# bobwan1995/cliora

Measured on AMD Instinct MI355X. Metric: sentences/sec (inside+outside fwd+bwd), len-20 d=400 bsz=64, higher is better.
Workload: dtype f32 (compose GEMMs: 3x bf16 MFMA per product, fp32 accumulate)

## Files before the change

cliora_amd/csrc/api_common.hpp:

```cpp
#pragma once
#include <hip/hip_runtime.h>
#include <hip/hip_ext.h>

#include <algorithm>
#include <cstdio>
#include <cstdlib>
#include <cstring>
#include <mutex>
#include <new>
#include <string>
#include <vector>

#include "../../include/cliora_chart.h"
#include "chart_kernels.hpp"
#include "gemm_kernels.hpp"
#include "wgrad_tiles.hpp"
#include "plan.hpp"

using namespace cliora;

struct cliora_plan {
    Plan p;
    bool uploaded = false;
    int device = -1;
// ... 170 lines not shown
enum { IMG_NONE = 0, IMG_FRAG_F32 = 2 };

template <class AP, class EP>
static int launch_rows_direct(hipStream_t st, const float* W, const float* img, int kind, int K, int ncols, int nrows, AP ap, EP ep) {
    if (nrows <= 0) return CLIORA_OK;
    const int nt = ncols / 16;
    if (kind == IMG_FRAG_F32) return launch_ksplit_f32<true>(st, img, K, nt, nrows, ap, ep);
    return launch_ksplit_f32<false>(st, W, K, nt, nrows, ap, ep);
}

template <class AP, class EP>
static int launch_rows(hipStream_t st, const float* W, int Kseg, int nseg, int ncols, int nrows, AP ap, EP ep) {
    if (nrows <= 0) return CLIORA_OK;
    const size_t budget = 150 * 1024;
    const int nt = ncols / 16;
    for (int ct : {5, 4, 2, 1}) {
        if (nt % ct) continue;
        if ((size_t)ct * 16 * (Kseg + WS_LDS_PAD) * sizeof(float) > budget) continue;
        switch (ct) {
            case 5: return launch_rows_ct<5>(st, W, Kseg, nseg, ncols, nrows, ap, ep);
            case 4: return launch_rows_ct<4>(st, W, Kseg, nseg, ncols, nrows, ap, ep);
            case 2: return launch_rows_ct<2>(st, W, Kseg, nseg, ncols, nrows, ap, ep);
            default: return launch_rows_ct<1>(st, W, Kseg, nseg, ncols, nrows, ap, ep);
        }
    }
    return fail(CLIORA_EINVAL, "weight block does not fit LDS");
}

constexpr int TN_DIRECT_ROWS = 4096;
constexpr int TN_DIRECT_BLOCKS = 256;

template <int T, class AP, class BP>
static int launch_tn_t(hipStream_t st, int nrows, int Mi, int Nj, AP ap, BP bp, float* slab, size_t slab_floats,
                       float* out, float* colsum_out, int accumulate) {
    const int blocks = (Mi / (T * 16)) * (Nj / (T * 16));
    size_t per_slice = (size_t)Mi * Nj + (colsum_out ? Mi : 0);
    int nsl = (int)std::min<size_t>(slab_floats / per_slice, (size_t)std::max(1, 2048 / blocks));
    nsl = std::min(nsl, (nrows + 15) / 16);
    nsl = std::max(4, nsl / 4 * 4);
    if ((size_t)nsl * per_slice > slab_floats) return fail(CLIORA_ENOMEM, "slab too small for the weight-gradient GEMM");
    int rps = (nrows + nsl - 1) / nsl;
    rps = (rps + 3) / 4 * 4;
    float* csl = slab + (size_t)nsl * Mi * Nj;
    if (colsum_out)
        hipLaunchKernelGGL((tn_gemm<T, T, true, AP, BP>), dim3(blocks, nsl / 4), dim3(WS_THREADS), 0, st, nrows, rps, Mi, Nj, ap, bp, slab, csl);
    else
        hipLaunchKernelGGL((tn_gemm<T, T, false, AP, BP>), dim3(blocks, nsl / 4), dim3(WS_THREADS), 0, st, nrows, rps, Mi, Nj, ap, bp, slab, csl);
    LAUNCHOK("tn_gemm");
    const size_t n = (size_t)Mi * Nj;
    launch_slab_reduce(st, slab, nsl, n, out, accumulate, csl, (size_t)Mi, colsum_out);
    LAUNCHOK("slab_reduce");
    return CLIORA_OK;
}

template <class AP, class BP>
static int launch_tn(hipStream_t st, int nrows, int Mi, int Nj, int Dp, AP ap, BP bp, float* slab, size_t slab_floats,
                     float* out, float* colsum_out, int accumulate = 0) {
    if (nrows <= 0) {
        if (accumulate) return CLIORA_OK;
        HIPOK(hipMemsetAsync(out, 0, (size_t)Mi * Nj * sizeof(float), st));
        if (colsum_out) HIPOK(hipMemsetAsync(colsum_out, 0, (size_t)Mi * sizeof(float), st));
        return CLIORA_OK;
    }
    if (nrows <= TN_DIRECT_ROWS && (Mi / 16) * (Nj / 16) <= TN_DIRECT_BLOCKS) {
        const int blocks = (Mi / 16) * (Nj / 16);
        if (colsum_out)
            hipLaunchKernelGGL((tn_gemm_direct<true, AP, BP>), dim3(blocks), dim3(TND_WAVES * 64), 0, st, nrows, Mi, Nj, ap, bp, out, colsum_out, accumulate);
        else
            hipLaunchKernelGGL((tn_gemm_direct<false, AP, BP>), dim3(blocks), dim3(TND_WAVES * 64), 0, st, nrows, Mi, Nj, ap, bp, out, colsum_out, accumulate);
        LAUNCHOK("tn_gemm_direct");
        return CLIORA_OK;
    }
    switch (pick_tiles(Dp / 16)) {
        case 5: return launch_tn_t<5>(st, nrows, Mi, Nj, ap, bp, slab, slab_floats, out, colsum_out, accumulate);
        case 4: return launch_tn_t<4>(st, nrows, Mi, Nj, ap, bp, slab, slab_floats, out, colsum_out, accumulate);
        case 2: return launch_tn_t<2>(st, nrows, Mi, Nj, ap, bp, slab, slab_floats, out, colsum_out, accumulate);
        default: return launch_tn_t<1>(st, nrows, Mi, Nj, ap, bp, slab, slab_floats, out, colsum_out, accumulate);
    }
}

template <int NIT, int NJT>
static int launch_tn_pairs_inst(hipStream_t st, const float* DZ, const float* X, int nrows, int Dp, int nkb, float* slab,
                                size_t slab_floats, float* out, float* colsum_out, int accumulate, int slices_cap, int ldz, int ldx) {
    const size_t per_slice = (size_t)Dp * Dp + Dp;
    int nsl = (int)std::min<size_t>(slab_floats / per_slice, (size_t)std::max(1, 256 / nkb));
    nsl = std::max(1, std::min(nsl, (nrows + 63) / 64));
    int rps = (nrows + nsl - 1) / nsl;
    rps = (rps + TN_RS - 1) / TN_RS * TN_RS;
    nsl = (nrows + rps - 1) / rps;
    float* csl = slab + (size_t)nsl * Dp * Dp;
    const size_t lds3 = (size_t)2 * TN3_RS * (Dp + NJT * 16) * sizeof(float) + (size_t)NJT * 2048;
    const bool strided = ldz != Dp || ldx != Dp;
    if (split_bf16() && lds3 <= 160 * 1024 && (Dp + NJT * 16) / 32 <= TN3_NP) {
        const int nsl_cap = slices_cap > 0 ? slices_cap : std::max(1, 230 / (8 * nkb)) * 8;
        if (nsl > nsl_cap) { nsl = nsl_cap; rps = (nrows + nsl - 1) / nsl; }
        rps = (rps + TN3_RS - 1) / TN3_RS * TN3_RS;
        nsl = (nrows + rps - 1) / rps;
        csl = slab + (size_t)nsl * Dp * Dp;
        if constexpr (NIT == 7 && NJT == 9) {
            OKR(cliora_ensure_max_lds((const void*)tn_gemm_dma3x<NIT, NJT, 5, true>));
            hipLaunchKernelGGL((tn_gemm_dma3x<NIT, NJT, 5, true>), dim3(8 * nkb * ((nsl + 7) / 8)), dim3(512), lds3, st, DZ, ldz, X, ldx, nrows, rps, nsl, Dp, Dp, nkb, slab, csl);
            LAUNCHOK("tn_gemm_dma3x");
        } else {
            if (strided) return fail(CLIORA_EINVAL, "strided operands need the eight-wave weight-gradient kernel (tn_pairs_strided_ok)");
            OKR(cliora_ensure_max_lds((const void*)tn_gemm_dma3<NIT, NJT, true>));
            hipLaunchKernelGGL((tn_gemm_dma3<NIT, NJT, true>), dim3(8 * nkb * ((nsl + 7) / 8)), dim3(256), lds3, st, DZ, X, nrows, rps, nsl, Dp, Dp, nkb, slab, csl);
            LAUNCHOK("tn_gemm_dma3");
        }
    } else {
        if (strided) return fail(CLIORA_EINVAL, "strided operands need the eight-wave weight-gradient kernel (tn_pairs_strided_ok)");
// ... 5 lines not shown
    const size_t n = (size_t)Dp * Dp;
    launch_slab_reduce(st, slab, nsl, n, out, accumulate, csl, (size_t)Dp, colsum_out);
    LAUNCHOK("slab_reduce");
    return CLIORA_OK;
}

static bool tn_pairs_two_ranges_ok(int Dp) {
    const int NT = Dp / 16;
    return split_bf16() && NT > 20 && NT <= 27;
}
static int launch_tn_pairs_two_ranges(hipStream_t st, const float* DZ, const float* X, int n1, long long start2, int n2, int Dp, float* slab,
                                      size_t slab_floats, float* out, float* colsum_out, int slices_cap) {
    constexpr int NIT = 7, NJT = 9, nkb = 3;
    const size_t per_slice = (size_t)Dp * Dp + Dp;
    const size_t lds3 = (size_t)2 * TN3_RS * (Dp + NJT * 16) * sizeof(float) + (size_t)NJT * 2048;
    int cap = std::min<int>((int)(slab_floats / per_slice), slices_cap > 0 ? slices_cap : std::max(1, 230 / (8 * nkb)) * 8);
    cap = std::max(2, cap);
    int rps = (n1 + n2 + cap - 1) / cap;
    rps = (rps + TN3_RS - 1) / TN3_RS * TN3_RS;
    int s1 = (n1 + rps - 1) / rps, s2 = (n2 + rps - 1) / rps;
    while (s1 + s2 > cap) { rps += TN3_RS; s1 = (n1 + rps - 1) / rps; s2 = (n2 + rps - 1) / rps; }
    const int nsl = s1 + s2;
    float* csl = slab + (size_t)nsl * Dp * Dp;
    OKR(cliora_ensure_max_lds((const void*)tn_gemm_dma3x<NIT, NJT, 5, true>));
    hipLaunchKernelGGL((tn_gemm_dma3x<NIT, NJT, 5, true>), dim3(8 * nkb * ((nsl + 7) / 8)), dim3(512), lds3, st, DZ, Dp, X, Dp, n1, rps, nsl, Dp, Dp, nkb,
                       slab, csl, s1, n2, start2);
    LAUNCHOK("tn_gemm_dma3x(two ranges)");
    launch_slab_reduce(st, slab, nsl, (size_t)Dp * Dp, out, 0, csl, (size_t)Dp, colsum_out);
    LAUNCHOK("slab_reduce");
    return CLIORA_OK;
}

static int launch_tn_level_block(hipStream_t st, const float* A, int lda, const float* Bm, int nsent, int C, int off, int hi, int Dp,
                                 float* slab, size_t slab_floats, float* out, float* colsum_out, int accumulate, int slices_cap, int nblk) {
    constexpr int NIT = 7, NJT = 9, nkb = 3;
    const int nrows = nsent * hi;
    if (nrows <= 0) return CLIORA_OK;
    const size_t per_slice = ((size_t)Dp * Dp + Dp) * nblk;
    const size_t lds3 = (size_t)2 * TN3_RS * (Dp + NJT * 16) * sizeof(float) + (size_t)NJT * 2048;
    int cap = std::min<int>((int)(slab_floats / per_slice), slices_cap > 0 ? slices_cap : std::max(1, 230 / (8 * nkb)) * 8);
    cap = std::max(1, std::min(cap, (nrows + 63) / 64));
    int rps = (nrows + cap - 1) / cap;
    rps = (rps + TN3_RS - 1) / TN3_RS * TN3_RS;
    const int nsl = (nrows + rps - 1) / rps;
    float* csl = slab + (size_t)nsl * nblk * Dp * Dp;
    OKR(cliora_ensure_max_lds((const void*)tn_gemm_dma3x<NIT, NJT, 5, true>));
    hipLaunchKernelGGL((tn_gemm_dma3x<NIT, NJT, 5, true>), dim3(8 * nkb * ((nsl + 7) / 8), nblk), dim3(512), lds3, st, A, lda, Bm, Dp, nrows, rps, nsl,
                       Dp, Dp, nkb, slab, csl, 0x7fffffff, 0, 0LL, hi, C, off, (long long)Dp);
    LAUNCHOK("tn_gemm_dma3x(level rows)");
    launch_slab_reduce(st, slab, nsl, (size_t)nblk * Dp * Dp, out, accumulate, csl, (size_t)nblk * Dp, colsum_out);
    LAUNCHOK("slab_reduce");
    return CLIORA_OK;
}

static bool pair_tiles_ok(int Dp) {
    return split_bf16() && Dp == 400;
}
static int launch_tn_tiles(hipStream_t st, const float* DZt, const float* Xt, long long tile0, long long ntiles, long long tile0b, long long ntilesb,
                           int Dp, float* slab, size_t slab_floats, float* out, float* colsum_out, int accumulate, int slices_cap) {
    const int NT = Dp / 16;
    const long long nt = ntiles + ntilesb;
    if (nt <= 0) {
        if (accumulate) return CLIORA_OK;
        HIPOK(hipMemsetAsync(out, 0, (size_t)Dp * Dp * sizeof(float), st));
        if (colsum_out) HIPOK(hipMemsetAsync(colsum_out, 0, (size_t)Dp * sizeof(float), st));
        return CLIORA_OK;
    }
    constexpr int NTc = 25, NIT = 7, NJT = 9, NJW = 5, nkb = 3;
    if (NT != NTc) return fail(CLIORA_EINVAL, "tiled pair-row operands: d = 400 only");
    const size_t per_slice = (size_t)Dp * Dp + Dp;
    long long cap = std::min<long long>((long long)(slab_floats / per_slice), slices_cap > 0 ? slices_cap : std::max(1, 230 / (8 * nkb)) * 8);
    cap = std::max<long long>(2, std::min(cap, (nt + 3) / 4));
    long long tps = (nt + cap - 1) / cap;
    tps = (tps + 1) / 2 * 2;
    long long s1 = (ntiles + tps - 1) / tps, s2 = (ntilesb + tps - 1) / tps;
    while (s1 + s2 > cap) { tps += 2; s1 = (ntiles + tps - 1) / tps; s2 = (ntilesb + tps - 1) / tps; }
    const int nsl = (int)(s1 + s2);
    float* csl = slab + (size_t)nsl * Dp * Dp;
    const size_t lds = (size_t)2 * 2048 * (NT + NJT) + 1024;
    OKR(cliora_ensure_max_lds((const void*)tn_gemm_tiles<NTc, NIT, NJT, NJW, true>));
    hipLaunchKernelGGL((tn_gemm_tiles<NTc, NIT, NJT, NJW, true>), dim3(8 * nkb * ((nsl + 7) / 8)), dim3(512), lds, st, reinterpret_cast<const uint32_t*>(DZt),
                       reinterpret_cast<const uint32_t*>(Xt), tile0, (int)ntiles, (int)tps, nsl, nkb, slab, csl, (int)s1, tile0b, (int)ntilesb);
// ... 198 lines not shown
```

cliora_amd/csrc/api_mlp.hip:

```cpp
#include "api_common.hpp"
#include <hip/hip_ext.h>
#include "level_kernels.hpp"
#include "ragged_kernels.hpp"
#include "resident_kernels.hpp"
#include "vl_kernels.hpp"

#define ATTEND_LAUNCH(kern, R_, grid, stream, ...)                                                              \
    do {                                                                                                      \
        if ((R_) <= 36) hipLaunchKernelGGL(kern<9>, grid, dim3(256), 0, stream, __VA_ARGS__);                  \
        else hipLaunchKernelGGL(kern<16>, grid, dim3(256), 0, stream, __VA_ARGS__);                            \
    } while (0)

struct ComposeLaunch { int TG, SP, ntask, gx; };
static ComposeLaunch compose_launch(const cliora_plan* plan, int level, bool outside_pass) {
    const Plan& p = plan->p;
    const int32_t* e = p.level_geom.data() + ((size_t)(outside_pass ? p.L : 0) + level) * PLEVEL_INTS;
    ComposeLaunch q{e[5], e[6], e[7], std::min(e[7], p.compose_cap)};
    if (q.gx >= 8 && (q.gx + 7) / 8 * 8 <= p.compose_cap) q.gx = (q.gx + 7) / 8 * 8;
    return q;
}

static size_t compose_lds_bytes(int ct, int S, bool with_slots) {
    return (size_t)ct * 16 * S * sizeof(uint32_t) + (with_slots ? (size_t)LC_SLOTS * ct * 64 * sizeof(float4) : 0);
}
// ... 680 lines not shown
        if (level == L - 1) {
            if (compress) {
                hipLaunchKernelGGL(cell_dnorm, dim3(cells_grid(ncell)), dim3(256), 0, sb, g, VHo, OH, ws + f.nrmo, p.normalize, dGo);
                LAUNCHOK("cell_dnorm(root)");
                return CLIORA_OK;
            }
            LAUNCH_SIGNALLING(done, root_bwd, dim3(1), dim3(ROOT_WAVES * 64), 0, sb, B, C, Dp, VHo, OH, ws + f.nrmo, p.normalize, wb + bw.groot);
            LAUNCHOK("root_bwd");
            return CLIORA_OK;
        }
        if (!fused_norm) {
            hipLaunchKernelGGL(cell_dnorm, dim3(cells_grid(ncell)), dim3(256), 0, sb, g, VHo, OH, ws + f.nrmo, p.normalize, dGo);
            LAUNCHOK("cell_dnorm(out)");
        }
        {
            ProfScope ps(CLIORA_KCLASS_COMPOSE_BWD, sb);
            OKR(launch_level_compose_bwd(sb, ws + f.w2oT, ws + f.w2oT3, f.S3, Dp, f.ct3, f.ncb3, pair_level(level, true), dGo, YM, Pp,
                                         PI + (size_t)p.blk_plo * Dp, ldpi, ws + f.po, Dp, ws + f.b2o, DA, DZ, Xp, DPP, DPB, tiled));
        }
        const bool sib_last = sibling_runs(L - 2 - level);
        LAUNCH_SIGNALLING(sib_last ? nullptr : done, cell_dsoftmax, dim3(cells_grid(ncell)), dim3(256), 0, sb, g, f.ncb3, DPP, DPB, Sp, Pp, OS, dStoto, DS);
        LAUNCHOK("cell_dsoftmax(out)");
        OKR(sibling_gather(L - 2 - level, done));
        return CLIORA_OK;
    };

    static const int ksplit_env = [] { const char* e = getenv("CLIORA_WGRAD_SPLIT_LEVEL"); return e ? atoi(e) : -1; }();
    const bool wcat_split_path = split_bf16() && tn_pairs_strided_ok(Dp);
    const bool sw_beside = plan->side2_beside;
    const int ksplit = ksplit_env >= 0 ? ksplit_env : !sw_beside ? 0
                     : wcat_split_path ? std::max(1, std::min(2 * L / 5, L - 1)) : std::min(2, L - 1);
    int tail_cells = C;
    bool dpi_done_recorded = false;
    auto wcat_grad = [&](hipStream_t s_, int off, int hi, int accumulate) -> int {
        if (tn_pairs_strided_ok(Dp) && (long long)B * hi >= 512 && (long long)B * hi < (1LL << 22)) {
            return launch_tn_level_block(s_, dPI, ldpi, IH, B, C, off, hi, Dp, wb + bw.slab2, bw.slab_floats, wb + bw.gwcat, wb + bw.gbcat, accumulate,
                                         std::max(8, (180 / (3 * nb)) / 4 * 4), nb);
        }
        return launch_tn(s_, B * hi, ldpi, Dp, Dp, LevelRowsA{dPI, ldpi, C, off, hi}, LevelRowsA{IH, Dp, C, off, hi}, wb + bw.slab2,
                         bw.slab_floats, wb + bw.gwcat, wb + bw.gbcat, accumulate);
    };
    auto inside_bwd_step = [&](int level) -> int {
        const LevelArgs g = level_args(p, level, false);
        const int ncell = B * g.Lc;
        const bool fused_norm = fuse_dnorm && p.share && !vl && level >= 1 && level <= L - 2;
        hipLaunchKernelGGL(cell_gather_bwd_in, dim3(ncell), dim3(256), 0, sa, g, D, d_inside_h,
                           level == 0 ? nullptr : d_inside_s, dv.use[ROLE_INA], dv.use[ROLE_INB], dv.use[ROLE_OUTA],
                           !ran_outside ? 0 : (sib_on_outside_chain(level) ? 1 : 2),
                           sibPL, sibQL, ldsib, wb + bw.sib_s, DA, DS, PI, ldpi, p.share, IH, OH, dPI, VH, dStot,
                           ws + f.bcat, fused_norm ? wb + bw.dots : nullptr);
        LAUNCHOK("cell_gather_bwd_in");
        if (level == 0) {
            HIPOK(hipEventRecord(plan->ev_fork[2], sa));
            dpi_done_recorded = true;
        }
        if (fused_norm && gemm3)
            OKR(launch_rows_direct3x(sa, ws + f.wcatT3s, ldpi, Dp, ncell, LevelRowsA{dPI, ldpi, C, g.off, g.Lc},
                              NormBwdLevelE{dG, VH, IH, ws + f.nrmi, wb + bw.dots, Dp, C, g.off, g.Lc, p.normalize}, bwd_gemm3));
        else if (fused_norm)
            OKR(launch_rows_direct(sa, ws + f.wcatT, PROJ_IMG(f.wcatT3), ldpi, Dp, ncell, LevelRowsA{dPI, ldpi, C, g.off, g.Lc},
                            NormBwdLevelE{dG, VH, IH, ws + f.nrmi, wb + bw.dots, Dp, C, g.off, g.Lc, p.normalize}));
        else if (level <= L - 2 && gemm3)
            OKR(launch_rows_direct3x(sa, ws + f.wcatT3s, ldpi, Dp, ncell, LevelRowsA{dPI, ldpi, C, g.off, g.Lc},
                              StoreLevelE{VH, Dp, C, g.off, g.Lc, nullptr, 1}, bwd_gemm3));
        else if (level <= L - 2)
            OKR(launch_rows_direct(sa, ws + f.wcatT, PROJ_IMG(f.wcatT3), ldpi, Dp, ncell, LevelRowsA{dPI, ldpi, C, g.off, g.Lc},
                            StoreLevelE{VH, Dp, C, g.off, g.Lc, nullptr, 1}));
        else if (compress && ran_outside)
            OKR(launch_rows_direct(sa, ws + f.rootwT, PROJ_IMG(f.rootwT3), Dp, Dp, ncell, LevelRowsA{dGo, Dp, C, g.off, g.Lc},
                            StoreLevelE{VH, Dp, C, g.off, g.Lc, nullptr, 1}));
        if (vl) {
            ATTEND_LAUNCH(cell_attend_bwd, p.R, dim3(ncell), sa, g, VH, IH, ws + f.nrmi, p.normalize, OBJ, p.R,
                               drop_mask, ws + f.att_pk, wb + bw.dctx, wb + bw.pmo, wb + bw.dsc, IHn, nrmIn, level >= 1 ? dG : (float*)nullptr);
            LAUNCHOK("cell_attend_bwd");
        }
        if (level == ksplit && level >= 1) {
            const int hi = tail_cells - g.off;
            HIPOK(hipEventRecord(plan->ev_fork[2], sa));
            HIPOK(hipStreamWaitEvent(sw, plan->ev_fork[2], 0));
            OKR(wcat_grad(sw, g.off, hi, tail_cells < C));
            tail_cells = g.off;
        }
        if (level == 0) return CLIORA_OK;
        if (!fused_norm && !vl) {
            hipLaunchKernelGGL(cell_dnorm, dim3(cells_grid(ncell)), dim3(256), 0, sa, g, VH, IHn, nrmIn, p.normalize, dG);
            LAUNCHOK("cell_dnorm(in)");
        }
        {
// ... 60 lines not shown
        }
        if (two_streams && j >= 1) HIPOK(hipStreamWaitEvent(sa, plan->ev_level[j - 1], 0));
        OKR(inside_bwd_step(L - 1 - j));
        if (j == J_early) {
            early_r0 = p.row_base_in(L - 1 - j);
            early_r1 = p.row_base_out(j + 1);
            HIPOK(hipEventRecord(plan->ev_fork[2], sa));
            HIPOK(hipStreamWaitEvent(sw, plan->ev_fork[2], 0));
            if (two_streams) HIPOK(hipStreamWaitEvent(sw, plan->ev_level[j], 0));
            early_t0 = p.tile_base_in(L - 1 - j);
            early_t1 = p.tile_base_out(j + 1);
            if (tiled)
                OKR(launch_tn_tiles(sw, DZ, Xp, early_t0, early_t1 - early_t0, 0, 0, Dp, wb + bw.slab2, bw.slab_floats, wb + bw.gw2o, wb + bw.gb2o, 0,
                                    early_slices));
            else
                OKR(launch_tn_pairs(sw, DZ + (size_t)early_r0 * Dp, Xp + (size_t)early_r0 * Dp, (int)(early_r1 - early_r0), Dp, wb + bw.slab2, bw.slab_floats,
                                    wb + bw.gw2o, wb + bw.gb2o, 0, early_slices));
        }
        if (tiled && J_early >= 0 && j == J_early2) {
            const long long t0 = p.tile_base_in(L - 1 - j), t1 = p.tile_base_out(j + 1);
            HIPOK(hipEventRecord(plan->ev_fork[2], sa));
            HIPOK(hipStreamWaitEvent(sw, plan->ev_fork[2], 0));
            if (two_streams) HIPOK(hipStreamWaitEvent(sw, plan->ev_level[j], 0));
            OKR(launch_tn_tiles(sw, DZ, Xp, t0, early_t0 - t0, early_t1, t1 - early_t1, Dp, wb + bw.slab2, bw.slab_floats, wb + bw.gw2o, wb + bw.gb2o, 1,
                                early_slices));
            early_t0 = t0; early_t1 = t1;
            early_r0 = p.row_base_in(L - 1 - j); early_r1 = p.row_base_out(j + 1);
        }
    }
    if (!resident) {
        hipLaunchKernelGGL(leaf_bwd_pre, dim3(cells_grid(B * L)), dim3(256), 0, st, B, L, C, Dp, VH, IHn, nrmIn, p.normalize, ws + f.t, dU);
        LAUNCHOK("leaf_bwd_pre");
    }
    if (d_x_span && !resident)
        OKR(launch_rows_direct(st, ws + f.wlT, PROJ_IMG(f.wlT3), Dp, Dp, B * L, PlainRowsA{dU, Dp}, StoreRowsE{d_x_span, D, nullptr, 0, D}));

    HIPOK(hipEventRecord(plan->ev_fork[1], st));
    constexpr int tail_slices = 48, tail_slices2 = 72;
    auto pair_rows_tail = [&](hipStream_t s_) -> int {
        ProfScope ps(CLIORA_KCLASS_WGRAD, s_);
        if (tiled) {
            if (ran_outside && !p.share)
                OKR(launch_tn_tiles(s_, DZ, Xp, p.T_in, p.T_out, 0, 0, Dp, wb + bw.slab, bw.slab_floats, wb + bw.gw2o, wb + bw.gb2o, 0, 0));
            const long long ntl = (p.share && ran_outside) ? p.T_in + p.T_out : p.T_in;
            if (J_early >= 0)
                OKR(launch_tn_tiles(s_, DZ, Xp, 0, early_t0, early_t1, ntl - early_t1, Dp, wb + bw.slab, bw.slab_floats, wb + bw.gw2i, wb + bw.gb2i, 0,
                                    tail_slices2));
            else
                OKR(launch_tn_tiles(s_, DZ, Xp, 0, ntl, 0, 0, Dp, wb + bw.slab, bw.slab_floats, wb + bw.gw2i, wb + bw.gb2i, 0, 0));
            return CLIORA_OK;
        }
        if (ran_outside && !p.share)
            OKR(launch_tn_pairs(s_, DZ + (size_t)p.R_in * Dp, Xp + (size_t)p.R_in * Dp, (int)p.R_out, Dp, wb + bw.slab, bw.slab_floats,
                                wb + bw.gw2o, wb + bw.gb2o));
        const long long nr = (p.share && ran_outside) ? p.R_in + p.R_out : p.R_in;
        if (J_early >= 0) {
            if (tn_pairs_two_ranges_ok(Dp))
                OKR(launch_tn_pairs_two_ranges(s_, DZ, Xp, (int)early_r0, early_r1, (int)(nr - early_r1), Dp, wb + bw.slab, bw.slab_floats,
                                               wb + bw.gw2i, wb + bw.gb2i, tail_slices2));
            else {
                OKR(launch_tn_pairs(s_, DZ, Xp, (int)early_r0, Dp, wb + bw.slab, bw.slab_floats, wb + bw.gw2i, wb + bw.gb2i, 0, tail_slices));
                OKR(launch_tn_pairs(s_, DZ + (size_t)early_r1 * Dp, Xp + (size_t)early_r1 * Dp, (int)(nr - early_r1), Dp, wb + bw.slab, bw.slab_floats,
                                    wb + bw.gw2i, wb + bw.gb2i, 1, tail_slices));
            }
        } else
            OKR(launch_tn_pairs(s_, DZ, Xp, (int)nr, Dp, wb + bw.slab, bw.slab_floats, wb + bw.gw2i, wb + bw.gb2i));
        return CLIORA_OK;
    };
    if (ran_outside) {
        if (two_streams) {
            if (tn_pairs_strided_ok(Dp))
                OKR(launch_tn_pairs(sb, dPO, OH, B * C, Dp, wb + bw.slab, bw.slab_floats, wb + bw.gw1ro, (float*)nullptr, 0, 72));
            else
                OKR(launch_tn(sb, B * C, Dp, Dp, Dp, PlainRowsA{dPO, Dp}, PlainRowsA{OH, Dp}, wb + bw.slab, bw.slab_floats, wb + bw.gw1ro,
                              (float*)nullptr));
            if (L >= 2) HIPOK(hipStreamWaitEvent(sb, plan->ev_join[2], 0));
            OKR(pair_rows_tail(sb));
            HIPOK(hipEventRecord(plan->ev_join[0], sb));
        } else {
            HIPOK(hipStreamWaitEvent(sw, plan->ev_fork[1], 0));
            if (tn_pairs_strided_ok(Dp))
                OKR(launch_tn_pairs(sw, dPO, OH, B * C, Dp, wb + bw.slab2, bw.slab_floats, wb + bw.gw1ro, (float*)nullptr, 0, 72));
            else
                OKR(launch_tn(sw, B * C, Dp, Dp, Dp, PlainRowsA{dPO, Dp}, PlainRowsA{OH, Dp}, wb + bw.slab2, bw.slab_floats, wb + bw.gw1ro,
                              (float*)nullptr));
        }
    }
    if (dpi_done_recorded) {
        HIPOK(hipStreamWaitEvent(sw, plan->ev_fork[2], 0));
        OKR(wcat_grad(sw, 0, tail_cells, tail_cells < C));
    }
    HIPOK(hipStreamWaitEvent(sw, plan->ev_fork[1], 0));
    if (vl && d_obj_span) {
        float* dO = padded ? wb + bw.dobjp : d_obj_span;
        if (Dp > 512) return fail(CLIORA_EINVAL, "obj_grad_reduce: D > 512 is not supported");
        if (p.R <= 36) {
            const size_t lds = (size_t)3 * 2 * 9 * 64 * sizeof(float4);
            OKR(cliora_ensure_max_lds((const void*)obj_grad_reduce<9>));
            hipLaunchKernelGGL(obj_grad_reduce<9>, dim3(B, 4), dim3(512), lds, sw, B, C, Dp, p.R, wb + bw.dctx, ws + f.att_u, wb + bw.pmo, wb + bw.dsc, dO);
        } else {
            const size_t lds = (size_t)3 * 2 * 16 * 64 * sizeof(float4);
            OKR(cliora_ensure_max_lds((const void*)obj_grad_reduce<16>));
            hipLaunchKernelGGL(obj_grad_reduce<16>, dim3(B, 4), dim3(512), lds, sw, B, C, Dp, p.R, wb + bw.dctx, ws + f.att_u, wb + bw.pmo, wb + bw.dsc, dO);
        }
        LAUNCHOK("obj_grad_reduce");
    }
    if (!dpi_done_recorded) OKR(wcat_grad(sw, 0, tail_cells, tail_cells < C));
    OKR(launch_tn(sw, B * L, Dp, Dp, Dp, PlainRowsA{dU, Dp}, PlainRowsA{X, Dp}, wb + bw.slab2, bw.slab_floats, wb + bw.gwl, wb + bw.gbl));
    HIPOK(hipEventRecord(plan->ev_join[1], sw));
    if (!two_streams) OKR(pair_rows_tail(st));
    else HIPOK(hipStreamWaitEvent(st, plan->ev_join[0], 0));
    HIPOK(hipStreamWaitEvent(st, plan->ev_join[1], 0));
    fork_guard.disarm();

    {
        CopyTable t; t.n = 0;
        const size_t DD = (size_t)Dp * Dp;
        if (vl && d_obj_span && padded) add_copy(t, d_obj_span, D, B * p.R, D, wb + bw.dobjp, Dp, B * p.R, D, 0, 0, 0);
        if (G->leaf_w) add_copy(t, G->leaf_w, D, D, D, wb + bw.gwl, Dp, D, D, 0, 0, 0);
        if (G->leaf_b) add_copy(t, G->leaf_b, D, 1, D, wb + bw.gbl, Dp, 1, D, 0, 0, 0);
        if (G->root_h && !compress) add_copy(t, G->root_h, D, 1, D, wb + bw.groot, Dp, 1, D, 0, 0, 0);
        if (G->root_mat && compress) add_copy(t, G->root_mat, D, D, D, wb + bw.groot_mat, Dp, D, D, 0, 0, 1);
        if (p.share) {
            if (G->in_w1) {
                add_copy(t, G->in_w1, 2 * D, D, D, wb + bw.gwcat, Dp, D, D, 0, 0, 0);
                add_copy(t, G->in_w1 + D, 2 * D, D, D, wb + bw.gwcat + DD, Dp, D, D, 0, 0, 0, wb + bw.gw1ro, Dp, D, D, 0, 0, 0);
            }
            if (G->in_b1) add_copy(t, G->in_b1, D, 1, D, wb + bw.gbcat, Dp, 1, D, 0, 0, 0);
            if (G->in_mat) add_copy(t, G->in_mat, D, D, D, wb + bw.gwcat + 2 * DD, Dp, D, D, 0, 0, 1);
            const float* gw2o_part = J_early >= 0 ? wb + bw.gw2o : nullptr;
            const float* gb2o_part = J_early >= 0 ? wb + bw.gb2o : nullptr;
            if (G->in_w2) add_copy(t, G->in_w2, D, D, D, wb + bw.gw2i, Dp, D, D, 0, 0, 0, gw2o_part, Dp, D, D, 0, 0, 0);
            if (G->in_b2) add_copy(t, G->in_b2, D, 1, D, wb + bw.gb2i, Dp, 1, D, 0, 0, 0, gb2o_part, Dp, 1, D, 0, 0, 0);
        } else {
            if (G->in_w1) {
                add_copy(t, G->in_w1, 2 * D, D, D, wb + bw.gwcat, Dp, D, D, 0, 0, 0);
                add_copy(t, G->in_w1 + D, 2 * D, D, D, wb + bw.gwcat + DD, Dp, D, D, 0, 0, 0);
            }
            if (G->in_b1) add_copy(t, G->in_b1, D, 1, D, wb + bw.gbcat, Dp, 1, D, 0, 0, 0);
            if (G->in_mat) add_copy(t, G->in_mat, D, D, D, wb + bw.gwcat + 2 * DD, Dp, D, D, 0, 0, 1);
            if (G->in_w2) add_copy(t, G->in_w2, D, D, D, wb + bw.gw2i, Dp, D, D, 0, 0, 0);
            if (G->in_b2) add_copy(t, G->in_b2, D, 1, D, wb + bw.gb2i, Dp, 1, D, 0, 0, 0);
// ... 14 lines not shown
```

cliora_amd/csrc/gemm_kernels.hpp:

```cpp
#pragma once
#include <hip/hip_runtime.h>
#include <stdint.h>

namespace cliora {

using f32x4 = __attribute__((ext_vector_type(4))) float;

__device__ __forceinline__ f32x4 mfma16(float a, float b, f32x4 c) {
    return __builtin_amdgcn_mfma_f32_16x16x4f32(a, b, c, 0, 0, 0);
}

template <int CTRL, int BANK>
__device__ __forceinline__ float wave_dpp(float old, float v) {
    return __int_as_float(__builtin_amdgcn_update_dpp(__float_as_int(old), __float_as_int(v), CTRL, 0xf, BANK, false));
}
template <class Op>
__device__ __forceinline__ float wave_butterfly(float v, Op op) {
    {
        auto r = __builtin_amdgcn_permlane32_swap(__float_as_uint(v), __float_as_uint(v), false, false);
        v = op(__uint_as_float(r[0]), __uint_as_float(r[1]));
    }
    {
        auto r = __builtin_amdgcn_permlane16_swap(__float_as_uint(v), __float_as_uint(v), false, false);
        v = op(__uint_as_float(r[0]), __uint_as_float(r[1]));
    }
    v = op(v, wave_dpp<0x128, 0xf>(v, v));
    { float t = wave_dpp<0x104, 0x5>(v, v); t = wave_dpp<0x114, 0xA>(t, v); v = op(v, t); }
    v = op(v, wave_dpp<0x4E, 0xf>(v, v));
    v = op(v, wave_dpp<0xB1, 0xf>(v, v));
    return v;
}
struct WaveAdd { __device__ __forceinline__ float operator()(float a, float b) const { return a + b; } };
struct WaveMax { __device__ __forceinline__ float operator()(float a, float b) const { return fmaxf(a, b); } };
__device__ __forceinline__ float wave_sum(float v) { return wave_butterfly(v, WaveAdd()); }
// ... 1182 lines not shown
                __builtin_amdgcn_sched_group_barrier(0x008, 1, 0);
                __builtin_amdgcn_sched_group_barrier(0x100, 1, 0);
                __builtin_amdgcn_sched_group_barrier(0x002, 1, 0);
            }
#pragma unroll
            for (int k = 8; k < 3 * NJW; ++k) {
                __builtin_amdgcn_sched_group_barrier(0x008, 1, 0);
                __builtin_amdgcn_sched_group_barrier(0x002, 2, 0);
                if (k - 8 < PPT) __builtin_amdgcn_sched_group_barrier(0x010, 1, 0);
            }
        }
    }
    float* out = slab + ((size_t)slice * nprob + prob) * Mi * Nj;
    if (has_tiles) {
#pragma unroll
        for (int t = 0; t < NIT; ++t)
            if (t < nit)
#pragma unroll
                for (int u = 0; u < NJW; ++u)
                    if (u < njw)
#pragma unroll
                        for (int reg = 0; reg < 4; ++reg)
                            out[(size_t)((it0 + t) * 16 + g * 4 + reg) * Nj + (jt0 + ju0 + u) * 16 + i] = acc[t][u][reg];
    }
    if (ones_here && has_tiles && i == 0) {
#pragma unroll
        for (int t = 0; t < NIT; ++t)
            if (t < nit)
#pragma unroll
                for (int reg = 0; reg < 4; ++reg) colsum[((size_t)slice * nprob + prob) * Mi + (it0 + t) * 16 + g * 4 + reg] = acc[t][NJW - 1][reg];
    }
}

template <int V>
static __global__ __launch_bounds__(256) void slab_reduce_k(const float* __restrict__ slab, int nslices, size_t n, float* __restrict__ out,
                                                            int accumulate, const float* __restrict__ csl, size_t ncs,
                                                            float* __restrict__ cs_out, unsigned nblk_main) {
    __shared__ float sh[3][64 * V];
    const int lane = threadIdx.x & 63, w = threadIdx.x >> 6;
    const bool main = blockIdx.x < nblk_main;
    const float* src = main ? slab : csl;
    float* dst = main ? out : cs_out;
    const size_t len = main ? n : ncs;
    const size_t e = ((size_t)(main ? blockIdx.x : blockIdx.x - nblk_main) * 64 + lane) * V;
    const bool ok = e < len;
    float acc[V];
#pragma unroll
    for (int v = 0; v < V; ++v) acc[v] = 0.f;
    if (ok) {
        for (int s0 = w; s0 < nslices; s0 += 32) {
            float t[8][V];
#pragma unroll
            for (int j = 0; j < 8; ++j) {
                const int s = s0 + 4 * j;
                const float* p = src + (size_t)min(s, nslices - 1) * len + e;
                if constexpr (V == 4) {
                    const float4 q = *reinterpret_cast<const float4*>(p);
                    t[j][0] = q.x; t[j][1] = q.y; t[j][2] = q.z; t[j][3] = q.w;
                } else {
                    t[j][0] = p[0];
                }
            }
#pragma unroll
            for (int j = 0; j < 8; ++j)
                if (s0 + 4 * j < nslices)
#pragma unroll
                    for (int v = 0; v < V; ++v) acc[v] += t[j][v];
        }
    }
    if (w > 0)
#pragma unroll
        for (int v = 0; v < V; ++v) sh[w - 1][lane * V + v] = acc[v];
    __syncthreads();
    if (w != 0 || !ok) return;
#pragma unroll
    for (int v = 0; v < V; ++v) {
        float r = (acc[v] + sh[0][lane * V + v]) + (sh[1][lane * V + v] + sh[2][lane * V + v]);
        if (accumulate) r += dst[e + v];
        acc[v] = r;
    }
    if constexpr (V == 4) *reinterpret_cast<float4*>(dst + e) = make_float4(acc[0], acc[1], acc[2], acc[3]);
    else dst[e] = acc[0];
}

static inline void launch_slab_reduce(hipStream_t st, const float* slab, int nslices, size_t n, float* out, int accumulate,
                                      const float* csl = nullptr, size_t ncs = 0, float* cs_out = nullptr) {
    if (!cs_out) ncs = 0;
    const bool vec = (n % 4 == 0) && (ncs % 4 == 0) && ((reinterpret_cast<uintptr_t>(slab) | reinterpret_cast<uintptr_t>(out) |
                                                        reinterpret_cast<uintptr_t>(csl) | reinterpret_cast<uintptr_t>(cs_out)) % 16 == 0);
    const int per = vec ? 256 : 64;
    const unsigned nb = (unsigned)((n + per - 1) / per), nc = (unsigned)((ncs + per - 1) / per);
    if (vec) hipLaunchKernelGGL(slab_reduce_k<4>, dim3(nb + nc), dim3(256), 0, st, slab, nslices, n, out, accumulate, csl, ncs, cs_out, nb);
    else hipLaunchKernelGGL(slab_reduce_k<1>, dim3(nb + nc), dim3(256), 0, st, slab, nslices, n, out, accumulate, csl, ncs, cs_out, nb);
}

}
```

cliora_amd/csrc/plan.cpp:

```cpp
#include "plan.hpp"

#include <algorithm>

namespace cliora {

static inline int ncells(int L) { return L * (L + 1) / 2; }

static size_t align64(size_t x) { return (x + 63) & ~size_t(63); }

ComposeGeom compose_geom(int ncell, int N, int cap) {
    const int G = (ncell + 15) / 16;
    ComposeGeom best{1, 1, G};
    double best_t = 1e30;
    for (int TG : {1, 2, 4, 8}) {
        const int wpg = 8 / TG;
        const int groups = (G + TG - 1) / TG;
        for (int SP = 1; SP <= HP_PARTS && SP <= std::max(1, N); SP *= 2) {
            const int np = (N + SP - 1) / SP;
            const int ntask = groups * SP;
            const int rounds = (ntask + cap - 1) / cap;
            const int depth = (np + wpg - 1) / wpg;
            const int busy = TG * std::min(wpg, np);
            int simd = depth * (busy > 4 ? 2 : 1);
            if (busy > 4 && wpg == 8 && np % 8 != 0 && np % 8 <= 4) simd -= 1;
// ... 172 lines not shown
        f.icp = take(lstm * BC * Dp); f.ocp = take(lstm * BC * Dp);
        f.nrmic = take(lstm * BC); f.nrmoc = take(lstm * BC); f.rootc = take(lstm * Dp);
        f.att_u = take(R > 0 ? BC * Dp : 0);
        f.att_pk = take(R > 0 ? BC * 64 : 0);
        f.att_nrmu = take(R > 0 ? BC : 0);
        f.rootw = take(arch == 0 ? Dp * Dp : 0); f.rootwT = take(arch == 0 ? Dp * Dp : 0);
        f.rootw3 = arch == 0 ? img(Dp, Dp) : o; f.rootwT3 = arch == 0 ? img(Dp, Dp) : o;
        f.rootpb = take(arch == 0 ? (size_t)B * Dp : 0);
        f.total = o;
        f.pair_h = arch == 0 ? o : f.y;
        f.pair_h_floats = arch == 0 ? align64(Rt * Dp) : 0;
    }
    {
        BwdLayout& b = p.bwd;
        size_t o = 0;
        auto take = [&](size_t n) { size_t at = o; o = align64(o + n); return at; };
        b.vh = take(BC * Dp); b.dg = take(BC * Dp); b.dstot = take(BC);
        b.vh_o = take(BC * Dp); b.dg_o = take(BC * Dp); b.dstot_o = take(BC);
        b.vc_o = take(lstm * BC * Dp); b.dgc_o = take(lstm * BC * Dp);
        b.da = take(lstm ? 0 : Rt * Dp); b.ds = take(Rt);
        const size_t Rtile = std::max(Rt, (size_t)(p.T_in + p.T_out) * 16);
        b.dz = take(lstm ? 0 : Rtile * Dp);
        b.x = take(arch == 0 ? Rtile * Dp : 0);
        b.dpp = take(arch == 0 ? Rt * p.fwd.ncb3 : 0);
        b.dpb = take(arch == 0 ? Rt : 0);
        b.dcb = take(0); b.vc = take(lstm * BC * Dp); b.dgc = take(lstm * BC * Dp); b.grootc = take(lstm * Dp);
        b.dpi = take(BC * nb * Dp); b.dpo = take(BC * npo * Dp);
        b.dots = take(arch == 0 ? BC : 0); b.dots_o = take(arch == 0 ? BC : 0);
        b.sib_pl = take((arch == 0 && p.share) ? BC * Dp : 0); b.sib_ql = take((arch == 0 && p.share) ? BC * Dp : 0); b.sib_s = take(arch == 0 ? BC : 0);
        b.du = take(BL * nlf * Dp); b.dxp = take(padded ? BL * Dp : 0);
        b.slab_floats = std::max((size_t)2048 * 80 * 80, (size_t)128 * (Dp * Dp + Dp));
        b.slab = take(b.slab_floats);
        b.slab2 = take(arch == 0 ? b.slab_floats : 0);
        b.gwcat = take(nb * Dp * Dp); b.gbcat = take(nb * Dp); b.gw1ro = take(npo * Dp * Dp);
        b.gw2i = take(Dp * Dp); b.gb2i = take(Dp); b.gw2o = take(Dp * Dp); b.gb2o = take(Dp);
        b.gwl = take(nlf * Dp * Dp); b.gbl = take(nlf * Dp); b.groot = take(Dp);
        b.dctx = take(R > 0 ? BC * Dp : 0);
        b.pmo = take(R > 0 ? BC * 64 : 0);
        b.dsc = take(R > 0 ? BC * 64 : 0);
        b.dobjp = take(R > 0 ? (size_t)B * R * Dp : 0);
        b.groot_mat = take(arch == 0 ? Dp * Dp : 0);
        b.total = o;
    }
    {
        auto& v = p.vl;
        size_t o = 0;
        auto take = [&](size_t n) { size_t at = o; o = align64(o + n); return at; };
        v.NRp = ((B * R + 15) / 16) * 16;
        const size_t NR = (size_t)v.NRp;
        const size_t on = R > 0 ? 1 : 0;
        v.oall = take(on * NR * Dp); v.oallT = take(on * NR * Dp);
        v.wall = take(on * NR * Dp); v.wallT = take(on * NR * Dp);
        v.sump = take(on * BC * Dp); v.xwp = take(on * BL * Dp); v.xwn = take(on * BL * Dp); v.dxn = take(on * BL * Dp); v.nrm = take(on * 4 * BL);
        v.gobj = take(on * NR * Dp);
        v.oimg = take(on * NR * ((Dp + 31) / 32 * 32 + 8));
        v.keys = take(on * 2 * (size_t)B * BC);
        v.slab_floats = on * (8 * (NR * Dp) + 64);
        v.slab = take(v.slab_floats);
        v.total = o;
    }
    p.compose_cap = std::max(1, (32 / std::max(1, p.fwd.ncb3))) * 8;
    if (p.fwd.ncb3 > 32) p.compose_cap = std::max(1, 256 / p.fwd.ncb3);
    p.level_geom.assign((size_t)2 * L * PLEVEL_INTS, 0);
    for (int pass = 0; pass < 2; ++pass)
        for (int lv = 0; lv < L; ++lv) {
            int32_t* e = p.level_geom.data() + ((size_t)pass * L + lv) * PLEVEL_INTS;
// ... 90 lines not shown
```

cliora_amd/csrc/plan.hpp:

```cpp
#pragma once
#include <cstddef>
#include <cstdint>
#include <string>
#include <vector>

namespace cliora {

constexpr int ROLE_INA = 0;
constexpr int ROLE_INB = 1;
constexpr int ROLE_OUTA = 2;
constexpr int ROLE_OUTB = 3;
constexpr int N_ROLES = 4;
constexpr int HP_PARTS = 4;
constexpr int CLIORA_MAX_L = 64;
constexpr int PLEVEL_INTS = 8;

struct UseList {
    std::vector<int32_t> off;
    std::vector<int32_t> row;
    std::vector<int32_t> stride;
    std::vector<int32_t> partner;
};

struct FwdLayout {
// ... 9 lines not shown
    size_t rootp;
    size_t rootw, rootwT, rootw3, rootwT3, rootpb;
    size_t matp, matq3, qrleaf;
    size_t xp, ihp, ohp;
    size_t objp;
    size_t t;
    size_t pi, po;
    size_t y, x;
    size_t pair_h;
    size_t pair_h_floats;
    size_t sp, pp;
    size_t hp, hp_o;
    size_t ymask;
    int ct3, ncb3;
    size_t nrmi, nrmo;
    size_t icp, ocp, nrmic, nrmoc, rootc;
    size_t att_u, att_pk, att_nrmu;
    size_t total;
};

struct BwdLayout {
    size_t vh, dg, dstot;
    size_t vh_o, dg_o, dstot_o;
    size_t vc_o, dgc_o;
    size_t da, ds;
    size_t dz;
    size_t x;
    size_t dpp, dpb;
    size_t dcb, vc, dgc, grootc;
    size_t dpi, dpo;
    size_t dots, dots_o;
    size_t sib_pl, sib_ql, sib_s;
    size_t du, dxp;
    size_t slab, slab2;
    size_t gwcat, gbcat, gw1ro, gw2i, gb2i, gw2o, gb2o, gwl, gbl, groot, groot_mat;
    size_t dctx, pmo, dsc, dobjp;
    size_t total;
    size_t slab_floats;
};

struct Plan {
    int B, L, D, Dp, C, share, normalize, R;
    int arch;
    int npo, nleaf;
    int off_pr, off_ql;
    int nblk;
    int blk_plo, blk_qlo;
    int P_in, P_out;
    long long R_in, R_out;
    std::vector<int32_t> level_offset;
    std::vector<int32_t> lvl_base_in, lvl_base_out;
    std::vector<int32_t> pair_a_in, pair_b_in;
    std::vector<int32_t> pair_a_out, pair_b_out;
    UseList uses[N_ROLES];
    std::vector<int32_t> arow, brow, trow;
    std::vector<int32_t> level_geom;
    int compose_cap;
    FwdLayout fwd;
    BwdLayout bwd;
    struct VlLayout { size_t oall, oallT, wall, wallT, sump, xwp, xwn, dxn, nrm, gobj, oimg, keys, slab, slab_floats, total; int NRp; } vl;

    int32_t* d_tables = nullptr;
    size_t d_tables_count = 0;
    struct DevOff { size_t pair_a_in, pair_b_in, pair_a_out, pair_b_out; size_t use_off[N_ROLES], use_row[N_ROLES], use_stride[N_ROLES], use_partner[N_ROLES]; size_t arow, brow, trow, lvl_base_in, lvl_base_out, level_geom; } dev;

    int Lc(int level) const { return L - level; }
    int Nin(int level) const { return level; }
// ... 22 lines not shown
```

Measured before the change: 22160.

## Move leaf weight-grad GEMM to main stream and merge slab reductions

In the non-resident path, the leaf weight-gradient GEMM now runs on the main stream before the fork, writing into a new third slab buffer. Its slab reduction is deferred and fused with the wcat weight-grad reduction into one combined kernel on the side stream. The join and fork events are signalled from the kernel launches themselves via hipExtLaunchKernelGGL instead of separate event records. The aim is fewer launches and better overlap between the two streams, at the cost of an extra slab allocation and more work on the main stream before the fork.

After: 22270, median of 6. No clear change (+0.5%).

```diff
diff --git a/cliora_amd/csrc/api_common.hpp b/cliora_amd/csrc/api_common.hpp
--- a/cliora_amd/csrc/api_common.hpp
+++ b/cliora_amd/csrc/api_common.hpp
@@ -226,7 +226,7 @@
 
 template <int T, class AP, class BP>
 static int launch_tn_t(hipStream_t st, int nrows, int Mi, int Nj, AP ap, BP bp, float* slab, size_t slab_floats,
-                       float* out, float* colsum_out, int accumulate) {
+                       float* out, float* colsum_out, int accumulate, SlabReduce* defer) {
     const int blocks = (Mi / (T * 16)) * (Nj / (T * 16));
     size_t per_slice = (size_t)Mi * Nj + (colsum_out ? Mi : 0);
     int nsl = (int)std::min<size_t>(slab_floats / per_slice, (size_t)std::max(1, 2048 / blocks));
@@ -242,6 +242,7 @@
         hipLaunchKernelGGL((tn_gemm<T, T, false, AP, BP>), dim3(blocks, nsl / 4), dim3(WS_THREADS), 0, st, nrows, rps, Mi, Nj, ap, bp, slab, csl);
     LAUNCHOK("tn_gemm");
     const size_t n = (size_t)Mi * Nj;
+    if (defer) { *defer = SlabReduce{slab, nsl, n, out, accumulate, csl, (size_t)Mi, colsum_out}; return CLIORA_OK; }
     launch_slab_reduce(st, slab, nsl, n, out, accumulate, csl, (size_t)Mi, colsum_out);
     LAUNCHOK("slab_reduce");
     return CLIORA_OK;
@@ -249,7 +250,7 @@
 
 template <class AP, class BP>
 static int launch_tn(hipStream_t st, int nrows, int Mi, int Nj, int Dp, AP ap, BP bp, float* slab, size_t slab_floats,
-                     float* out, float* colsum_out, int accumulate = 0) {
+                     float* out, float* colsum_out, int accumulate = 0, SlabReduce* defer = nullptr) {
     if (nrows <= 0) {
         if (accumulate) return CLIORA_OK;
         HIPOK(hipMemsetAsync(out, 0, (size_t)Mi * Nj * sizeof(float), st));
@@ -266,10 +267,10 @@
         return CLIORA_OK;
     }
     switch (pick_tiles(Dp / 16)) {
-        case 5: return launch_tn_t<5>(st, nrows, Mi, Nj, ap, bp, slab, slab_floats, out, colsum_out, accumulate);
-        case 4: return launch_tn_t<4>(st, nrows, Mi, Nj, ap, bp, slab, slab_floats, out, colsum_out, accumulate);
-        case 2: return launch_tn_t<2>(st, nrows, Mi, Nj, ap, bp, slab, slab_floats, out, colsum_out, accumulate);
-        default: return launch_tn_t<1>(st, nrows, Mi, Nj, ap, bp, slab, slab_floats, out, colsum_out, accumulate);
+        case 5: return launch_tn_t<5>(st, nrows, Mi, Nj, ap, bp, slab, slab_floats, out, colsum_out, accumulate, defer);
+        case 4: return launch_tn_t<4>(st, nrows, Mi, Nj, ap, bp, slab, slab_floats, out, colsum_out, accumulate, defer);
+        case 2: return launch_tn_t<2>(st, nrows, Mi, Nj, ap, bp, slab, slab_floats, out, colsum_out, accumulate, defer);
+        default: return launch_tn_t<1>(st, nrows, Mi, Nj, ap, bp, slab, slab_floats, out, colsum_out, accumulate, defer);
     }
 }
 
@@ -341,7 +342,8 @@
 }
 
 static int launch_tn_level_block(hipStream_t st, const float* A, int lda, const float* Bm, int nsent, int C, int off, int hi, int Dp,
-                                 float* slab, size_t slab_floats, float* out, float* colsum_out, int accumulate, int slices_cap, int nblk) {
+                                 float* slab, size_t slab_floats, float* out, float* colsum_out, int accumulate, int slices_cap, int nblk,
+                                 SlabReduce* defer = nullptr) {
     constexpr int NIT = 7, NJT = 9, nkb = 3;
     const int nrows = nsent * hi;
     if (nrows <= 0) return CLIORA_OK;
@@ -357,6 +359,7 @@
     hipLaunchKernelGGL((tn_gemm_dma3x<NIT, NJT, 5, true>), dim3(8 * nkb * ((nsl + 7) / 8), nblk), dim3(512), lds3, st, A, lda, Bm, Dp, nrows, rps, nsl,
                        Dp, Dp, nkb, slab, csl, 0x7fffffff, 0, 0LL, hi, C, off, (long long)Dp);
     LAUNCHOK("tn_gemm_dma3x(level rows)");
+    if (defer) { *defer = SlabReduce{slab, nsl, (size_t)nblk * Dp * Dp, out, accumulate, csl, (size_t)nblk * Dp, colsum_out}; return CLIORA_OK; }
     launch_slab_reduce(st, slab, nsl, (size_t)nblk * Dp * Dp, out, accumulate, csl, (size_t)nblk * Dp, colsum_out);
     LAUNCHOK("slab_reduce");
     return CLIORA_OK;
diff --git a/cliora_amd/csrc/api_mlp.hip b/cliora_amd/csrc/api_mlp.hip
--- a/cliora_amd/csrc/api_mlp.hip
+++ b/cliora_amd/csrc/api_mlp.hip
@@ -736,28 +736,25 @@
                      : wcat_split_path ? std::max(1, std::min(2 * L / 5, L - 1)) : std::min(2, L - 1);
     int tail_cells = C;
     bool dpi_done_recorded = false;
-    auto wcat_grad = [&](hipStream_t s_, int off, int hi, int accumulate) -> int {
+    auto wcat_grad = [&](hipStream_t s_, int off, int hi, int accumulate, SlabReduce* defer = nullptr) -> int {
         if (tn_pairs_strided_ok(Dp) && (long long)B * hi >= 512 && (long long)B * hi < (1LL << 22)) {
             return launch_tn_level_block(s_, dPI, ldpi, IH, B, C, off, hi, Dp, wb + bw.slab2, bw.slab_floats, wb + bw.gwcat, wb + bw.gbcat, accumulate,
-                                         std::max(8, (180 / (3 * nb)) / 4 * 4), nb);
+                                         std::max(8, (180 / (3 * nb)) / 4 * 4), nb, defer);
         }
         return launch_tn(s_, B * hi, ldpi, Dp, Dp, LevelRowsA{dPI, ldpi, C, off, hi}, LevelRowsA{IH, Dp, C, off, hi}, wb + bw.slab2,
-                         bw.slab_floats, wb + bw.gwcat, wb + bw.gbcat, accumulate);
+                         bw.slab_floats, wb + bw.gwcat, wb + bw.gbcat, accumulate, defer);
     };
     auto inside_bwd_step = [&](int level) -> int {
         const LevelArgs g = level_args(p, level, false);
         const int ncell = B * g.Lc;
         const bool fused_norm = fuse_dnorm && p.share && !vl && level >= 1 && level <= L - 2;
-        hipLaunchKernelGGL(cell_gather_bwd_in, dim3(ncell), dim3(256), 0, sa, g, D, d_inside_h,
+        LAUNCH_SIGNALLING(level == 0 ? plan->ev_fork[2] : (hipEvent_t) nullptr, cell_gather_bwd_in, dim3(ncell), dim3(256), 0, sa, g, D, d_inside_h,
                            level == 0 ? nullptr : d_inside_s, dv.use[ROLE_INA], dv.use[ROLE_INB], dv.use[ROLE_OUTA],
                            !ran_outside ? 0 : (sib_on_outside_chain(level) ? 1 : 2),
                            sibPL, sibQL, ldsib, wb + bw.sib_s, DA, DS, PI, ldpi, p.share, IH, OH, dPI, VH, dStot,
                            ws + f.bcat, fused_norm ? wb + bw.dots : nullptr);
         LAUNCHOK("cell_gather_bwd_in");
-        if (level == 0) {
-            HIPOK(hipEventRecord(plan->ev_fork[2], sa));
-            dpi_done_recorded = true;
-        }
+        if (level == 0) dpi_done_recorded = true;
         if (fused_norm && gemm3)
             OKR(launch_rows_direct3x(sa, ws + f.wcatT3s, ldpi, Dp, ncell, LevelRowsA{dPI, ldpi, C, g.off, g.Lc},
                               NormBwdLevelE{dG, VH, IH, ws + f.nrmi, wb + bw.dots, Dp, C, g.off, g.Lc, p.normalize}, bwd_gemm3));
@@ -884,10 +881,14 @@
         hipLaunchKernelGGL(leaf_bwd_pre, dim3(cells_grid(B * L)), dim3(256), 0, st, B, L, C, Dp, VH, IHn, nrmIn, p.normalize, ws + f.t, dU);
         LAUNCHOK("leaf_bwd_pre");
     }
+    SlabReduce leaf_red, wcat_red;
+    SlabReduce* const wcat_defer = resident ? nullptr : &wcat_red;
+    if (!resident)
+        OKR(launch_tn(st, B * L, Dp, Dp, Dp, PlainRowsA{dU, Dp}, PlainRowsA{X, Dp}, wb + bw.slab3, bw.slab_floats, wb + bw.gwl, wb + bw.gbl, 0, &leaf_red));
+    HIPOK(hipEventRecord(plan->ev_fork[1], st));
     if (d_x_span && !resident)
         OKR(launch_rows_direct(st, ws + f.wlT, PROJ_IMG(f.wlT3), Dp, Dp, B * L, PlainRowsA{dU, Dp}, StoreRowsE{d_x_span, D, nullptr, 0, D}));
 
-    HIPOK(hipEventRecord(plan->ev_fork[1], st));
     constexpr int tail_slices = 48, tail_slices2 = 72;
     auto pair_rows_tail = [&](hipStream_t s_) -> int {
         ProfScope ps(CLIORA_KCLASS_WGRAD, s_);
@@ -940,7 +941,7 @@
     }
     if (dpi_done_recorded) {
         HIPOK(hipStreamWaitEvent(sw, plan->ev_fork[2], 0));
-        OKR(wcat_grad(sw, 0, tail_cells, tail_cells < C));
+        OKR(wcat_grad(sw, 0, tail_cells, tail_cells < C, wcat_defer));
     }
     HIPOK(hipStreamWaitEvent(sw, plan->ev_fork[1], 0));
     if (vl && d_obj_span) {
@@ -957,9 +958,15 @@
         }
         LAUNCHOK("obj_grad_reduce");
     }
-    if (!dpi_done_recorded) OKR(wcat_grad(sw, 0, tail_cells, tail_cells < C));
-    OKR(launch_tn(sw, B * L, Dp, Dp, Dp, PlainRowsA{dU, Dp}, PlainRowsA{X, Dp}, wb + bw.slab2, bw.slab_floats, wb + bw.gwl, wb + bw.gbl));
-    HIPOK(hipEventRecord(plan->ev_join[1], sw));
+    if (!dpi_done_recorded) OKR(wcat_grad(sw, 0, tail_cells, tail_cells < C, wcat_defer));
+    if (resident) {
+        OKR(launch_tn(sw, B * L, Dp, Dp, Dp, PlainRowsA{dU, Dp}, PlainRowsA{X, Dp}, wb + bw.slab2, bw.slab_floats, wb + bw.gwl, wb + bw.gbl));
+        HIPOK(hipEventRecord(plan->ev_join[1], sw));
+    } else {
+        const bool signalled = launch_slab_reduce2(sw, wcat_red, leaf_red, plan->ev_join[1]);
+        LAUNCHOK("slab_reduce2");
+        if (!signalled) HIPOK(hipEventRecord(plan->ev_join[1], sw));
+    }
     if (!two_streams) OKR(pair_rows_tail(st));
     else HIPOK(hipStreamWaitEvent(st, plan->ev_join[0], 0));
     HIPOK(hipStreamWaitEvent(st, plan->ev_join[1], 0));
diff --git a/cliora_amd/csrc/gemm_kernels.hpp b/cliora_amd/csrc/gemm_kernels.hpp
--- a/cliora_amd/csrc/gemm_kernels.hpp
+++ b/cliora_amd/csrc/gemm_kernels.hpp
@@ -1,5 +1,6 @@
 #pragma once
 #include <hip/hip_runtime.h>
+#include <hip/hip_ext.h>
 #include <stdint.h>
 
 namespace cliora {
@@ -1248,17 +1249,23 @@
     }
 }
 
+struct SlabReduce {
+    const float* slab = nullptr;
+    int nslices = 0;
+    size_t n = 0;
+    float* out = nullptr;
+    int accumulate = 0;
+    const float* csl = nullptr;
+    size_t ncs = 0;
+    float* cs_out = nullptr;
+    bool pending() const { return slab != nullptr; }
+};
+
 template <int V>
-static __global__ __launch_bounds__(256) void slab_reduce_k(const float* __restrict__ slab, int nslices, size_t n, float* __restrict__ out,
-                                                            int accumulate, const float* __restrict__ csl, size_t ncs,
-                                                            float* __restrict__ cs_out, unsigned nblk_main) {
-    __shared__ float sh[3][64 * V];
+static __device__ __forceinline__ void slab_reduce_block(const float* __restrict__ src, int nslices, size_t len, float* __restrict__ dst,
+                                                         int accumulate, size_t blk, float (*sh)[64 * V]) {
     const int lane = threadIdx.x & 63, w = threadIdx.x >> 6;
-    const bool main = blockIdx.x < nblk_main;
-    const float* src = main ? slab : csl;
-    float* dst = main ? out : cs_out;
-    const size_t len = main ? n : ncs;
-    const size_t e = ((size_t)(main ? blockIdx.x : blockIdx.x - nblk_main) * 64 + lane) * V;
+    const size_t e = (blk * 64 + lane) * V;
     const bool ok = e < len;
     float acc[V];
 #pragma unroll
@@ -1299,15 +1306,69 @@
     else dst[e] = acc[0];
 }
 
+template <int V>
+static __global__ __launch_bounds__(256) void slab_reduce_k(const float* __restrict__ slab, int nslices, size_t n, float* __restrict__ out,
+                                                            int accumulate, const float* __restrict__ csl, size_t ncs,
+                                                            float* __restrict__ cs_out, unsigned nblk_main) {
+    __shared__ float sh[3][64 * V];
+    const bool main = blockIdx.x < nblk_main;
+    slab_reduce_block<V>(main ? slab : csl, nslices, main ? n : ncs, main ? out : cs_out, accumulate,
+                         main ? blockIdx.x : blockIdx.x - nblk_main, sh);
+}
+
+template <int V>
+static __global__ __launch_bounds__(256) void slab_reduce2_k(SlabReduce a, unsigned a_main, unsigned a_all, SlabReduce b, unsigned b_main) {
+    __shared__ float sh[3][64 * V];
+    const bool first = blockIdx.x < a_all;
+    const SlabReduce& r = first ? a : b;
+    const unsigned blk = first ? blockIdx.x : blockIdx.x - a_all;
+    const bool main = blk < (first ? a_main : b_main);
+    slab_reduce_block<V>(main ? r.slab : r.csl, r.nslices, main ? r.n : r.ncs, main ? r.out : r.cs_out, r.accumulate,
+                         main ? blk : blk - (first ? a_main : b_main), sh);
+}
+
+static inline bool slab_reduce_vec_ok(const float* slab, size_t n, float* out, const float* csl, size_t ncs, float* cs_out) {
+    return (n % 4 == 0) && (ncs % 4 == 0) && ((reinterpret_cast<uintptr_t>(slab) | reinterpret_cast<uintptr_t>(out) |
+                                               reinterpret_cast<uintptr_t>(csl) | reinterpret_cast<uintptr_t>(cs_out)) % 16 == 0);
+}
+
 static inline void launch_slab_reduce(hipStream_t st, const float* slab, int nslices, size_t n, float* out, int accumulate,
-                                      const float* csl = nullptr, size_t ncs = 0, float* cs_out = nullptr) {
+                                      const float* csl = nullptr, size_t ncs = 0, float* cs_out = nullptr, hipEvent_t done = nullptr) {
     if (!cs_out) ncs = 0;
-    const bool vec = (n % 4 == 0) && (ncs % 4 == 0) && ((reinterpret_cast<uintptr_t>(slab) | reinterpret_cast<uintptr_t>(out) |
-                                                        reinterpret_cast<uintptr_t>(csl) | reinterpret_cast<uintptr_t>(cs_out)) % 16 == 0);
+    const bool vec = slab_reduce_vec_ok(slab, n, out, csl, ncs, cs_out);
     const int per = vec ? 256 : 64;
     const unsigned nb = (unsigned)((n + per - 1) / per), nc = (unsigned)((ncs + per - 1) / per);
+    if (done) {
+        if (vec) hipExtLaunchKernelGGL(slab_reduce_k<4>, dim3(nb + nc), dim3(256), 0, st, nullptr, done, 0, slab, nslices, n, out, accumulate, csl, ncs, cs_out, nb);
+        else hipExtLaunchKernelGGL(slab_reduce_k<1>, dim3(nb + nc), dim3(256), 0, st, nullptr, done, 0, slab, nslices, n, out, accumulate, csl, ncs, cs_out, nb);
+        return;
+    }
     if (vec) hipLaunchKernelGGL(slab_reduce_k<4>, dim3(nb + nc), dim3(256), 0, st, slab, nslices, n, out, accumulate, csl, ncs, cs_out, nb);
     else hipLaunchKernelGGL(slab_reduce_k<1>, dim3(nb + nc), dim3(256), 0, st, slab, nslices, n, out, accumulate, csl, ncs, cs_out, nb);
 }
 
-}
+static inline bool launch_slab_reduce2(hipStream_t st, SlabReduce a, SlabReduce b, hipEvent_t done = nullptr) {
+    if (!a.pending() && !b.pending()) return false;
+    if (!a.pending() || !b.pending()) {
+        const SlabReduce& r = a.pending() ? a : b;
+        launch_slab_reduce(st, r.slab, r.nslices, r.n, r.out, r.accumulate, r.csl, r.ncs, r.cs_out, done);
+        return true;
+    }
+    if (!a.cs_out) a.ncs = 0;
+    if (!b.cs_out) b.ncs = 0;
+    const bool vec = slab_reduce_vec_ok(a.slab, a.n, a.out, a.csl, a.ncs, a.cs_out) && slab_reduce_vec_ok(b.slab, b.n, b.out, b.csl, b.ncs, b.cs_out);
+    const int per = vec ? 256 : 64;
+    const unsigned am = (unsigned)((a.n + per - 1) / per), ac = (unsigned)((a.ncs + per - 1) / per);
+    const unsigned bm = (unsigned)((b.n + per - 1) / per), bc = (unsigned)((b.ncs + per - 1) / per);
+    const dim3 grid(am + ac + bm + bc);
+    if (done) {
+        if (vec) hipExtLaunchKernelGGL(slab_reduce2_k<4>, grid, dim3(256), 0, st, nullptr, done, 0, a, am, am + ac, b, bm);
+        else hipExtLaunchKernelGGL(slab_reduce2_k<1>, grid, dim3(256), 0, st, nullptr, done, 0, a, am, am + ac, b, bm);
+    } else {
+        if (vec) hipLaunchKernelGGL(slab_reduce2_k<4>, grid, dim3(256), 0, st, a, am, am + ac, b, bm);
+        else hipLaunchKernelGGL(slab_reduce2_k<1>, grid, dim3(256), 0, st, a, am, am + ac, b, bm);
+    }
+    return true;
+}
+
+}
diff --git a/cliora_amd/csrc/plan.cpp b/cliora_amd/csrc/plan.cpp
--- a/cliora_amd/csrc/plan.cpp
+++ b/cliora_amd/csrc/plan.cpp
@@ -228,6 +228,7 @@
         b.slab_floats = std::max((size_t)2048 * 80 * 80, (size_t)128 * (Dp * Dp + Dp));
         b.slab = take(b.slab_floats);
         b.slab2 = take(arch == 0 ? b.slab_floats : 0);
+        b.slab3 = take(arch == 0 ? b.slab_floats : 0);
         b.gwcat = take(nb * Dp * Dp); b.gbcat = take(nb * Dp); b.gw1ro = take(npo * Dp * Dp);
         b.gw2i = take(Dp * Dp); b.gb2i = take(Dp); b.gw2o = take(Dp * Dp); b.gb2o = take(Dp);
         b.gwl = take(nlf * Dp * Dp); b.gbl = take(nlf * Dp); b.groot = take(Dp);
diff --git a/cliora_amd/csrc/plan.hpp b/cliora_amd/csrc/plan.hpp
--- a/cliora_amd/csrc/plan.hpp
+++ b/cliora_amd/csrc/plan.hpp
@@ -65,7 +65,7 @@
     size_t dots, dots_o;
     size_t sib_pl, sib_ql, sib_s;
     size_t du, dxp;
-    size_t slab, slab2;
+    size_t slab, slab2, slab3;
     size_t gwcat, gbcat, gw1ro, gw2i, gb2i, gw2o, gb2o, gwl, gbl, groot, groot_mat;
     size_t dctx, pmo, dsc, dobjp;
     size_t total;
```
